# KRLabsOrg/verbatim-rag

Hardware: AMD Instinct MI355X
Metric: query x chunk span-extractions/sec @512tok (ModernBERT-base extractor, chunks/s) (higher is better)
Workload: dtype bf16

## Files before the change

verbatim-rag_amd/csrc/qkv_attn.hip:

```cpp
#include "qkv_attn.h"

#include <cstdlib>
#include <type_traits>

#ifdef VRAG_DEBUG_API
#define VRAG_DBG(bit) ((p.debug_flags & (bit)) != 0)
#else
#define VRAG_DBG(bit) false
#endif

namespace vrag {

constexpr int QA_WB = 192 * 128;
constexpr int QA_XOFF = 2 * QA_WB;
constexpr int QA_TAB = 131072;
constexpr int QA_MU = QA_TAB, QA_RS = QA_TAB + 2048, QA_LS = QA_TAB + 4096;
constexpr int QA_CA = QA_TAB + 5120, QA_SA = QA_CA + 4096, QA_CB = QA_SA + 4096, QA_SB = QA_CB + 2048;
constexpr int QA_SMEM = QA_SB + 2048;
constexpr int QA_V_OFF = 65536;

constexpr float QA_LAZY = 8.0f;
__device__ __forceinline__ float max3f(float a, float b, float c) { return __builtin_fmaxf(__builtin_fmaxf(a, b), c); }

template <int N>
__device__ __forceinline__ void wait_vm() {
  asm volatile("s_waitcnt vmcnt(%0)" ::"n"(N) : "memory");
}

template <bool LOCAL, bool FOLD, typename T>
__global__ __launch_bounds__(512, 2) void qkv_attn_kernel(const QkvAttnParams p) {
  typedef typename Op<T>::v4 V4;
  typedef typename Op<T>::v8 V8;
  extern __shared__ __attribute__((aligned(16))) char smem[];
  const int tid = threadIdx.x;
  const int lane = tid & 63;
  const int wave = uniform(tid >> 6);
  const int g = lane >> 4, l15 = lane & 15;
  const int H = p.H, Tp = p.Tp, nh = p.nh;
  const int xcd = blockIdx.x & 7, slot = blockIdx.x >> 3;
  const int grp = (slot / nh) * 8 + xcd, head = slot % nh;
  if (grp >= p.n_groups) return;
  const int4 wd = p.groups[grp * 8 + wave];
  const int wrow0 = uniform(wd.x), S = uniform(wd.y), kbase = uniform(wd.z);
  const int srow0 = wave * 64;
  const int qrow0 = (wave - kbase) * 64;
  const bool active = qrow0 < S;
  const T* X = reinterpret_cast<const T*>(p.x);
  const T* Wh = reinterpret_cast<const T*>(p.w) + (size_t)head * 192 * H;

  unsigned voffX[2], voffW[3];
#pragma unroll
  for (int par = 0; par < 2; ++par) {
    const int r = par * 8 + (lane >> 3);
    voffX[par] = (unsigned)(r * H + (((lane & 7) ^ ((r >> 1) & 7)) << 3)) * 2u;
  }
#pragma unroll
  for (int i = 0; i < 3; ++i) {
    const int row = wave * 24 + i * 8 + (lane >> 3);
    voffW[i] = (unsigned)(row * H + (((lane & 7) ^ ((row >> 1) & 7)) << 3)) * 2u;
  }
  const char* const Xw = reinterpret_cast<const char*>(X + (size_t)wrow0 * H);
  const char* const Wb = reinterpret_cast<const char*>(Wh);
  char* const xbuf = smem + QA_XOFF + wave * 8192;
  auto dma_w = [&](int kt, int buf, int i) {
    if (VRAG_DBG(4)) return;
    unsigned vo = voffW[i];
    asm volatile("" : "+v"(vo));
    glds16(Wb + kt * 128 + vo, smem + buf * QA_WB + (wave * 24 + i * 8) * 128);
  };
  auto dma_x = [&](int kt, int i) {
    if (!active || VRAG_DBG(4)) return;
    unsigned vo = voffX[i & 1];
    asm volatile("" : "+v"(vo));
    glds16(Xw + ((size_t)(i >> 1) * 16 * H + kt * 64) * 2 + vo, xbuf + i * 1024);
  };

  if (!VRAG_DBG(4)) {
    if (FOLD && lane < 16) {
      glds16(p.ln_mu + min(wrow0 + lane * 4, Tp - 4), smem + QA_MU + srow0 * 4);
      glds16(p.ln_rstd + min(wrow0 + lane * 4, Tp - 4), smem + QA_RS + srow0 * 4);
    }
    if (FOLD && wave == 2) glds16(p.ln_s + head * 192 + lane * 4, smem + QA_LS);
    if (wave == 2 || wave == 3) {
      const float* tab = wave == 2 ? p.rope_cos : p.rope_sin;
#pragma unroll
      for (int i = 0; i < 2; ++i) {
        const int r = i * 8 + (lane >> 3);
        glds16(tab + min(r, p.rope_rows - 1) * 32 + (((lane & 7) ^ ((r >> 1) & 7)) << 2), smem + (wave == 2 ? QA_CB : QA_SB) + i * 1024);
      }
    }
    if (wave == 4 || wave == 5) {
      const float* tab = wave == 4 ? p.rope_cos : p.rope_sin;
#pragma unroll
      for (int i = 0; i < 4; ++i)
        glds16(tab + (size_t)min(16 * (i * 8 + (lane >> 3)), p.rope_rows - 1) * 32 + (lane & 7) * 4, smem + (wave == 4 ? QA_CA : QA_SA) + i * 1024);
    }
  }

  f32x4 acc[12][4];
#pragma unroll
  for (int a = 0; a < 12; ++a)
#pragma unroll
    for (int c = 0; c < 4; ++c) acc[a][c] = f32x4{0.f, 0.f, 0.f, 0.f};

  const int KT = H >> 6;
  int fo[2];
#pragma unroll
  for (int s2 = 0; s2 < 2; ++s2) fo[s2] = l15 * 128 + ((((4 * s2 + g) ^ ((l15 >> 1) & 7))) << 4);
#ifdef VRAG_DEBUG_API
  const int probe = p.debug_flags;
#else
  int probe = 0;
  asm volatile("" : "+s"(probe));
#endif
  const bool mm = active && !(probe & 2);
#pragma unroll
  for (int i = 0; i < 3; ++i) dma_w(0, 0, i);
#pragma unroll
  for (int i = 0; i < 8; ++i) dma_x(0, i);
  for (int kt = 0; kt < KT; ++kt) {
    wait_vm<0>();
    __builtin_amdgcn_s_barrier();
    asm volatile("" ::: "memory");
    const char* sW = smem + (kt & 1) * QA_WB;
    const bool more = kt + 1 < KT;
    V8 xf[2][4], wa;
    if (mm) {
#pragma unroll
      for (int s2 = 0; s2 < 2; ++s2)
#pragma unroll
        for (int rt = 0; rt < 4; ++rt) xf[s2][rt] = *reinterpret_cast<const V8*>(xbuf + rt * 16 * 128 + fo[s2]);
      wa = *reinterpret_cast<const V8*>(sW + fo[0]);
    }
    asm volatile("s_waitcnt lgkmcnt(0)" ::: "memory");
    __builtin_amdgcn_sched_barrier(0);
    if (mm) {
#pragma unroll
      for (int it = 0; it < 24; ++it) {
        const int s2 = it / 12, nj = it % 12;
        V8 na = wa;
        if (it < 23) na = *reinterpret_cast<const V8*>(sW + ((it + 1) % 12) * 16 * 128 + fo[(it + 1) / 12]);
        __builtin_amdgcn_sched_barrier(0);
#pragma unroll
        for (int rt = 0; rt < 4; ++rt) {
          if (nj < 8) acc[nj][rt] = Op<T>::mfma16(wa, xf[s2][rt], acc[nj][rt]);
          else acc[nj][rt] = Op<T>::mfma16(xf[s2][rt], wa, acc[nj][rt]);
        }
        __builtin_amdgcn_sched_barrier(0);
        if (more && it < 11) {
          if (it < 3) dma_w(kt + 1, (kt + 1) & 1, it);
          else dma_x(kt + 1, it - 3);
        }
        __builtin_amdgcn_sched_barrier(0);
        wa = na;
      }
    } else if (more) {
#pragma unroll
      for (int i = 0; i < 3; ++i) dma_w(kt + 1, (kt + 1) & 1, i);
#pragma unroll
      for (int i = 0; i < 8; ++i) dma_x(kt + 1, i);
    }
  }
  __syncthreads();
  if (VRAG_DBG(16)) return;

  const float* l_mu = reinterpret_cast<const float*>(smem + QA_MU) + srow0;
  const float* l_rs = reinterpret_cast<const float*>(smem + QA_RS) + srow0;
  const float* l_ls = reinterpret_cast<const float*>(smem + QA_LS);
#pragma unroll
  for (int db = 0; db < 4; ++db) {
    const int d = db * 16 + l15;
    const float lsv = FOLD ? l_ls[128 + d] : 0.f;
#pragma unroll
    for (int tp = 0; tp < 2; ++tp) {
      V8 vv;
#pragma unroll
      for (int a = 0; a < 2; ++a) {
        const int rt = 2 * tp + a;
        f32x4 m4 = {0.f, 0.f, 0.f, 0.f}, r4 = {1.f, 1.f, 1.f, 1.f};
        if constexpr (FOLD) {
          m4 = *reinterpret_cast<const f32x4*>(l_mu + rt * 16 + 4 * g);
          r4 = *reinterpret_cast<const f32x4*>(l_rs + rt * 16 + 4 * g);
        }
#pragma unroll
        for (int h = 0; h < 2; ++h) {
          const int r0 = 2 * h;
          const f32x2 v = pk_fma(f32x2{-m4[r0], -m4[r0 + 1]}, splat2(lsv), f32x2{acc[8 + db][rt][r0], acc[8 + db][rt][r0 + 1]}) * f32x2{r4[r0], r4[r0 + 1]};
#pragma unroll
          for (int e = 0; e < 2; ++e)
            vv[a * 4 + r0 + e] = qrow0 + rt * 16 + 4 * g + r0 + e < S ? Op<T>::to(v[e]) : (T)0.f;
        }
      }
      const int c = wave * 8 + tp * 4 + g;
      *reinterpret_cast<V8*>(smem + QA_V_OFF + d * 1024 + ((c ^ l15) << 4)) = vv;
    }
  }
  auto rope_rows = [&](int a0, int rt, int ls_off, float scale, V8 (&out)[2]) {
    const bool live = qrow0 + rt * 16 + l15 < S;
    const float mu = FOLD ? l_mu[rt * 16 + l15] : 0.f, rs = FOLD ? l_rs[rt * 16 + l15] : 1.f;
#pragma unroll
    for (int np = 0; np < 2; ++np) {
      const int dd = np * 16 + 4 * g;
      const f32x4 ca = *reinterpret_cast<const f32x4*>(smem + QA_CA + (((qrow0 >> 4) + rt) * 32 + dd) * 4);
      const f32x4 sa = *reinterpret_cast<const f32x4*>(smem + QA_SA + (((qrow0 >> 4) + rt) * 32 + dd) * 4);
      const int bsw = l15 * 128 + ((((dd >> 2) ^ ((l15 >> 1) & 7))) << 4);
      const f32x4 cb = *reinterpret_cast<const f32x4*>(smem + QA_CB + bsw);
      const f32x4 sb = *reinterpret_cast<const f32x4*>(smem + QA_SB + bsw);
      f32x4 l1 = {0.f, 0.f, 0.f, 0.f}, l2 = {0.f, 0.f, 0.f, 0.f};
      if constexpr (FOLD) {
        l1 = *reinterpret_cast<const f32x4*>(l_ls + ls_off + dd);
        l2 = *reinterpret_cast<const f32x4*>(l_ls + ls_off + 32 + dd);
      }
#pragma unroll
      for (int h = 0; h < 2; ++h) {
        const int j0 = 2 * h;
        f32x2 x1 = {acc[a0 + np][rt][j0], acc[a0 + np][rt][j0 + 1]}, x2 = {acc[a0 + 2 + np][rt][j0], acc[a0 + 2 + np][rt][j0 + 1]};
        if constexpr (FOLD) {
          x1 = pk_fma(splat2(-mu), f32x2{l1[j0], l1[j0 + 1]}, x1) * rs;
          x2 = pk_fma(splat2(-mu), f32x2{l2[j0], l2[j0 + 1]}, x2) * rs;
        }
        const f32x2 ca2 = {ca[j0], ca[j0 + 1]}, sa2 = {sa[j0], sa[j0 + 1]}, cb2 = {cb[j0], cb[j0 + 1]}, sb2 = {sb[j0], sb[j0 + 1]};
        const f32x2 c = pk_fma(-sa2, sb2, ca2 * cb2), sn = pk_fma(ca2, sb2, sa2 * cb2);
        const f32x2 o1 = pk_fma(-x2, sn, x1 * c) * scale, o2 = pk_fma(x1, sn, x2 * c) * scale;
#pragma unroll
        for (int e = 0; e < 2; ++e) {
          if constexpr (!std::is_same<T, bf16_t>::value) {
            out[0][np * 4 + j0 + e] = live ? Op<T>::to(o1[e]) : (T)0.f;
            out[1][np * 4 + j0 + e] = live ? Op<T>::to(o2[e]) : (T)0.f;
          } else {
            out[0][np * 4 + j0 + e] = Op<T>::to(o1[e]);
            out[1][np * 4 + j0 + e] = Op<T>::to(o2[e]);
          }
        }
      }
    }
  };
#pragma unroll
  for (int rt = 0; rt < 4; ++rt) {
    V8 kf[2];
    rope_rows(4, rt, 64, 1.0f, kf);
    const int row = srow0 + rt * 16 + l15;
#pragma unroll
    for (int s = 0; s < 2; ++s) *reinterpret_cast<V8*>(smem + row * 128 + (((4 * s + g) ^ ((row >> 1) & 7)) << 4)) = kf[s];
  }
  V8 qf[4][2];
#pragma unroll
  for (int rt = 0; rt < 4; ++rt) rope_rows(0, rt, 0, p.q_scale, qf[rt]);
  __syncthreads();

  f32x4 ot[4][4];
  f32x4 lo[4];
#pragma unroll
  for (int c = 0; c < 4; ++c) {
    lo[c] = f32x4{0.f, 0.f, 0.f, 0.f};
#pragma unroll
    for (int dt = 0; dt < 4; ++dt) ot[c][dt] = f32x4{0.f, 0.f, 0.f, 0.f};
  }
  float m_run[4] = {0.f, 0.f, 0.f, 0.f};
  bool seen[4] = {false, false, false, false};
  V8 ones;
#pragma unroll
  for (int j = 0; j < 8; ++j) ones[j] = (T)1.0f;
  const int W = p.window;
  int kt_lo = 0, kt_hi = (S - 1) >> 6;
  if constexpr (LOCAL) {
    kt_lo = max(0, qrow0 - W) >> 6;
    kt_hi = min(S - 1, qrow0 + 63 + W) >> 6;
  }
  const int ksw = (l15 >> 1) & 7;
  if (active && !VRAG_DBG(1)) {
    for (int kt = kt_lo; kt <= kt_hi; ++kt) {
      bool cut[2][2];
#pragma unroll
      for (int u = 0; u < 2; ++u) {
        const int q_lo = qrow0 + 32 * u;
#pragma unroll
        for (int t2 = 0; t2 < 2; ++t2) {
          const int kh = kt * 64 + t2 * 32;
          bool outside = kh >= S || q_lo >= S;
          cut[u][t2] = kh + 31 >= S;
          if constexpr (LOCAL) {
            outside = outside || (kh + 31 < q_lo - W) || (kh > q_lo + 31 + W);
            cut[u][t2] = cut[u][t2] || (kh < q_lo + 31 - W) || (kh + 31 > q_lo + W);
          }
          cut[u][t2] = cut[u][t2] || outside;
        }
      }
      V8 pf[4][2];
      {
        f32x4 st[4][4];
#pragma unroll
        for (int c = 0; c < 4; ++c) {
          const float seed = -m_run[c];
#pragma unroll
          for (int kb = 0; kb < 4; ++kb) st[c][kb] = f32x4{seed, seed, seed, seed};
        }
#pragma unroll
        for (int kb = 0; kb < 4; ++kb) {
          const char* krow = smem + ((kbase + kt) * 64 + kb * 16 + l15) * 128;
          const V8 k0 = *reinterpret_cast<const V8*>(krow + ((g ^ ksw) << 4));
          const V8 k1 = *reinterpret_cast<const V8*>(krow + (((4 + g) ^ ksw) << 4));
#pragma unroll
          for (int c = 0; c < 4; ++c) {
            st[c][kb] = Op<T>::mfma16(k0, qf[c][0], st[c][kb]);
            st[c][kb] = Op<T>::mfma16(k1, qf[c][1], st[c][kb]);
          }
        }
        float mx[4];
#pragma unroll
        for (int c = 0; c < 4; ++c) {
          const int u = c >> 1;
          mx[c] = -INFINITY;
#pragma unroll
          for (int t2 = 0; t2 < 2; ++t2) {
            if (cut[u][t2]) {
              const int qi = qrow0 + 16 * c + l15;
              int lo_k = 0, hi_k = S - 1;
              if constexpr (LOCAL) {
                lo_k = max(0, qi - W);
                hi_k = min(S - 1, qi + W);
              }
              const unsigned span = hi_k >= lo_k ? (unsigned)(hi_k - lo_k) : 0u;
              int d0 = hi_k >= lo_k ? kt * 64 + t2 * 32 + 4 * g - lo_k : -100000;
              asm volatile("" : "+v"(d0));
#pragma unroll
              for (int h2 = 0; h2 < 2; ++h2)
#pragma unroll
                for (int r = 0; r < 4; ++r) {
                  const bool ok = (unsigned)(d0 + 16 * h2 + r) <= span;
                  st[c][2 * t2 + h2][r] = ok ? st[c][2 * t2 + h2][r] : -INFINITY;
                }
            }
            const f32x4& a = st[c][2 * t2];
            const f32x4& b2 = st[c][2 * t2 + 1];
            mx[c] = max3f(mx[c], max3f(a[0], a[1], a[2]), max3f(a[3], b2[0], b2[1]));
            mx[c] = max3f(mx[c], b2[2], b2[3]);
          }
        }
        bool move = false;
#pragma unroll
        for (int c = 0; c < 4; ++c) move = move || mx[c] > QA_LAZY || (!seen[c] && mx[c] > -INFINITY);
        if (__any(move)) {
#pragma unroll
          for (int c = 0; c < 4; ++c) {
            float m_all = fmaxf(mx[c], __shfl_xor(mx[c], 16, 64));
            m_all = fmaxf(m_all, __shfl_xor(m_all, 32, 64));
            const bool has = m_all > -INFINITY;
            const float delta = seen[c] ? fmaxf(m_all, 0.f) : (has ? m_all : 0.f);
            const float alpha = seen[c] ? __builtin_amdgcn_exp2f(-delta) : 1.0f;
            seen[c] = seen[c] || has;
            m_run[c] += delta;
#pragma unroll
            for (int kb = 0; kb < 4; ++kb)
#pragma unroll
              for (int r = 0; r < 4; ++r) st[c][kb][r] -= delta;
#pragma unroll
            for (int dt = 0; dt < 4; ++dt)
#pragma unroll
              for (int r = 0; r < 4; ++r) ot[c][dt][r] *= alpha;
#pragma unroll
            for (int r = 0; r < 4; ++r) lo[c][r] *= alpha;
          }
        }
#pragma unroll
        for (int c = 0; c < 4; ++c)
#pragma unroll
          for (int t2 = 0; t2 < 2; ++t2)
#pragma unroll
            for (int j = 0; j < 8; ++j) pf[c][t2][j] = (T)__builtin_amdgcn_exp2f(st[c][2 * t2 + (j >> 2)][j & 3]);
      }
#pragma unroll
      for (int t2 = 0; t2 < 2; ++t2) {
#pragma unroll
        for (int c = 0; c < 4; ++c) lo[c] = Op<T>::mfma16(ones, pf[c][t2], lo[c]);
#pragma unroll
        for (int dt = 0; dt < 4; ++dt) {
          const V8 vf = *reinterpret_cast<const V8*>(smem + QA_V_OFF + (dt * 16 + l15) * 1024 + ((((kbase + kt) * 8 + t2 * 4 + g) ^ l15) << 4));
#pragma unroll
          for (int c = 0; c < 4; ++c) ot[c][dt] = Op<T>::mfma16(vf, pf[c][t2], ot[c][dt]);
        }
      }
    }
  }
  __syncthreads();

  if (active) {
    char* stg = smem + wave * 8192;
#pragma unroll
    for (int rt = 0; rt < 4; ++rt) {
      const int row = rt * 16 + l15;
      const bool live = qrow0 + row < S;
      const float inv = live ? 1.0f / lo[rt][0] : 0.f;
#pragma unroll
      for (int db = 0; db < 4; ++db) {
        V4 o;
#pragma unroll
        for (int j = 0; j < 4; ++j) o[j] = live ? Op<T>::to(ot[rt][db][j] * inv) : (T)0.f;
        const int c16 = db * 2 + (g >> 1);
        *reinterpret_cast<V4*>(stg + row * 128 + ((c16 ^ (row & 7)) << 4) + ((g & 1) << 3)) = o;
      }
    }
#pragma unroll
    for (int it = 0; it < 8; ++it) {
      const int row = it * 8 + (lane >> 3), c16 = lane & 7;
      const f32x4 v = *reinterpret_cast<const f32x4*>(stg + row * 128 + ((c16 ^ (row & 7)) << 4));
      if (qrow0 + row < S && !VRAG_DBG(8)) store16_nt(reinterpret_cast<T*>(p.o) + (size_t)(wrow0 + row) * H + head * 64 + c16 * 8, v);
    }
  }
}

template <bool LOCAL, bool FOLD, typename T>
static hipError_t launch_t(const QkvAttnParams& p, hipStream_t stream) {
  static bool attr = false;
  if (!attr) {
    hipError_t e = hipFuncSetAttribute(reinterpret_cast<const void*>(&qkv_attn_kernel<LOCAL, FOLD, T>),
                                       hipFuncAttributeMaxDynamicSharedMemorySize, QA_SMEM);
    if (e != hipSuccess) return e;
    attr = true;
  }
  const int grid = ((p.n_groups + 7) / 8) * 8 * p.nh;
  hipLaunchKernelGGL((qkv_attn_kernel<LOCAL, FOLD, T>), dim3(grid), dim3(512), QA_SMEM, stream, p);
  return hipGetLastError();
}

hipError_t launch_qkv_attention(const QkvAttnParams& p, bool local, hipStream_t stream) {
  if (p.n_groups <= 0) return hipSuccess;
  if (p.H % 64 != 0 || p.H != p.nh * 64 || (size_t)p.Tp * p.H >= (size_t)1 << 31) return hipErrorInvalidValue;
  const bool fold = p.ln_mu != nullptr;
  if (p.op_dtype == kOpF16) {
    if (fold) return local ? launch_t<true, true, f16_t>(p, stream) : launch_t<false, true, f16_t>(p, stream);
    return local ? launch_t<true, false, f16_t>(p, stream) : launch_t<false, false, f16_t>(p, stream);
  }
  if (fold) return local ? launch_t<true, true, bf16_t>(p, stream) : launch_t<false, true, bf16_t>(p, stream);
  return local ? launch_t<true, false, bf16_t>(p, stream) : launch_t<false, false, bf16_t>(p, stream);
}

__global__ void permute_qkv_heads_kernel(const bf16_t* __restrict__ w, const float* __restrict__ s, int H, int nh,
                                         bf16_t* __restrict__ w_out, float* __restrict__ s_out) {
  const int orow = blockIdx.x;
  const int head = orow / 192, part = (orow % 192) / 64, d = orow % 64;
  const int src = part * H + head * 64 + d;
  for (int i = threadIdx.x; i < H; i += blockDim.x) w_out[(size_t)orow * H + i] = w[(size_t)src * H + i];
  if (threadIdx.x == 0 && s && s_out) s_out[orow] = s[src];
}

hipError_t permute_qkv_heads(const bf16_t* w, const float* s, int H, int nh, bf16_t* w_out, float* s_out, hipStream_t stream) {
  hipLaunchKernelGGL(permute_qkv_heads_kernel, dim3(3 * H), dim3(256), 0, stream, w, s, H, nh, w_out, s_out);
  return hipGetLastError();
}

int fused_pack_groups(const int* seq_row, const int* seq_len, int seq0, int seq1, int4* out) {
  int n = 0, used = 8;
  for (int s = seq0; s < seq1; ++s) {
    const int need = (seq_len[s] + 63) / 64;
    if (used + need > 8) {
      for (int w = 0; w < 8; ++w) out[n * 8 + w] = int4{0, 0, 0, 0};
      ++n;
      used = 0;
    }
    for (int j = 0; j < need; ++j) out[(n - 1) * 8 + used + j] = int4{seq_row[s] + 64 * j, seq_len[s], used, 0};
    used += need;
  }
  return n;
}

unsigned qkv_attn_f16_saturated(bool reset) { return f16_sat_take(reset); }
unsigned* qkv_attn_f16_flag_address() { return f16_sat_flag_address(); }

}
```

Before: 7633.

## Skip dead attention sub-blocks at local-window edges and specialize full-tile epilogue

Splits the key-tile loop in local (sliding-window) attention so the first and last tiles use compile-time specializations that skip MFMA, masking, exp and PV work for 32x32 sub-blocks entirely outside the window. The V/K/Q rope epilogue is also templated on whether the query tile is fully in-bounds, removing per-element bounds selects for full bf16 folded tiles, and the q scale is folded into the row scale multiply. This adds code size and register pressure from multiple instantiations.

```diff
diff --git a/verbatim-rag_amd/csrc/qkv_attn.hip b/verbatim-rag_amd/csrc/qkv_attn.hip
--- a/verbatim-rag_amd/csrc/qkv_attn.hip
+++ b/verbatim-rag_amd/csrc/qkv_attn.hip
@@ -167,85 +167,93 @@
   const float* l_mu = reinterpret_cast<const float*>(smem + QA_MU) + srow0;
   const float* l_rs = reinterpret_cast<const float*>(smem + QA_RS) + srow0;
   const float* l_ls = reinterpret_cast<const float*>(smem + QA_LS);
-#pragma unroll
-  for (int db = 0; db < 4; ++db) {
-    const int d = db * 16 + l15;
-    const float lsv = FOLD ? l_ls[128 + d] : 0.f;
-#pragma unroll
-    for (int tp = 0; tp < 2; ++tp) {
-      V8 vv;
-#pragma unroll
-      for (int a = 0; a < 2; ++a) {
-        const int rt = 2 * tp + a;
-        f32x4 m4 = {0.f, 0.f, 0.f, 0.f}, r4 = {1.f, 1.f, 1.f, 1.f};
+  V8 qf[4][2];
+  auto epilogue = [&](auto all_c) __attribute__((always_inline)) {
+    constexpr bool ALL = decltype(all_c)::value;
+#pragma unroll
+    for (int db = 0; db < 4; ++db) {
+      const int d = db * 16 + l15;
+      const float lsv = FOLD ? l_ls[128 + d] : 0.f;
+#pragma unroll
+      for (int tp = 0; tp < 2; ++tp) {
+        V8 vv;
+#pragma unroll
+        for (int a = 0; a < 2; ++a) {
+          const int rt = 2 * tp + a;
+          f32x4 m4 = {0.f, 0.f, 0.f, 0.f}, r4 = {1.f, 1.f, 1.f, 1.f};
+          if constexpr (FOLD) {
+            m4 = *reinterpret_cast<const f32x4*>(l_mu + rt * 16 + 4 * g);
+            r4 = *reinterpret_cast<const f32x4*>(l_rs + rt * 16 + 4 * g);
+          }
+#pragma unroll
+          for (int h = 0; h < 2; ++h) {
+            const int r0 = 2 * h;
+            const f32x2 v = pk_fma(f32x2{-m4[r0], -m4[r0 + 1]}, splat2(lsv), f32x2{acc[8 + db][rt][r0], acc[8 + db][rt][r0 + 1]}) * f32x2{r4[r0], r4[r0 + 1]};
+#pragma unroll
+            for (int e = 0; e < 2; ++e)
+              vv[a * 4 + r0 + e] = ALL || qrow0 + rt * 16 + 4 * g + r0 + e < S ? Op<T>::to(v[e]) : (T)0.f;
+          }
+        }
+        const int c = wave * 8 + tp * 4 + g;
+        *reinterpret_cast<V8*>(smem + QA_V_OFF + d * 1024 + ((c ^ l15) << 4)) = vv;
+      }
+    }
+    auto rope_rows = [&](int a0, int rt, int ls_off, float scale, V8 (&out)[2]) {
+      const bool live = ALL || qrow0 + rt * 16 + l15 < S;
+      const float mu = FOLD ? l_mu[rt * 16 + l15] : 0.f, rs = FOLD ? l_rs[rt * 16 + l15] * scale : scale;
+#pragma unroll
+      for (int np = 0; np < 2; ++np) {
+        const int dd = np * 16 + 4 * g;
+        const f32x4 ca = *reinterpret_cast<const f32x4*>(smem + QA_CA + (((qrow0 >> 4) + rt) * 32 + dd) * 4);
+        const f32x4 sa = *reinterpret_cast<const f32x4*>(smem + QA_SA + (((qrow0 >> 4) + rt) * 32 + dd) * 4);
+        const int bsw = l15 * 128 + ((((dd >> 2) ^ ((l15 >> 1) & 7))) << 4);
+        const f32x4 cb = *reinterpret_cast<const f32x4*>(smem + QA_CB + bsw);
+        const f32x4 sb = *reinterpret_cast<const f32x4*>(smem + QA_SB + bsw);
+        f32x4 l1 = {0.f, 0.f, 0.f, 0.f}, l2 = {0.f, 0.f, 0.f, 0.f};
         if constexpr (FOLD) {
-          m4 = *reinterpret_cast<const f32x4*>(l_mu + rt * 16 + 4 * g);
-          r4 = *reinterpret_cast<const f32x4*>(l_rs + rt * 16 + 4 * g);
+          l1 = *reinterpret_cast<const f32x4*>(l_ls + ls_off + dd);
+          l2 = *reinterpret_cast<const f32x4*>(l_ls + ls_off + 32 + dd);
         }
 #pragma unroll
         for (int h = 0; h < 2; ++h) {
-          const int r0 = 2 * h;
-          const f32x2 v = pk_fma(f32x2{-m4[r0], -m4[r0 + 1]}, splat2(lsv), f32x2{acc[8 + db][rt][r0], acc[8 + db][rt][r0 + 1]}) * f32x2{r4[r0], r4[r0 + 1]};
-#pragma unroll
-          for (int e = 0; e < 2; ++e)
-            vv[a * 4 + r0 + e] = qrow0 + rt * 16 + 4 * g + r0 + e < S ? Op<T>::to(v[e]) : (T)0.f;
-        }
-      }
-      const int c = wave * 8 + tp * 4 + g;
-      *reinterpret_cast<V8*>(smem + QA_V_OFF + d * 1024 + ((c ^ l15) << 4)) = vv;
-    }
-  }
-  auto rope_rows = [&](int a0, int rt, int ls_off, float scale, V8 (&out)[2]) {
-    const bool live = qrow0 + rt * 16 + l15 < S;
-    const float mu = FOLD ? l_mu[rt * 16 + l15] : 0.f, rs = FOLD ? l_rs[rt * 16 + l15] : 1.f;
-#pragma unroll
-    for (int np = 0; np < 2; ++np) {
-      const int dd = np * 16 + 4 * g;
-      const f32x4 ca = *reinterpret_cast<const f32x4*>(smem + QA_CA + (((qrow0 >> 4) + rt) * 32 + dd) * 4);
-      const f32x4 sa = *reinterpret_cast<const f32x4*>(smem + QA_SA + (((qrow0 >> 4) + rt) * 32 + dd) * 4);
-      const int bsw = l15 * 128 + ((((dd >> 2) ^ ((l15 >> 1) & 7))) << 4);
-      const f32x4 cb = *reinterpret_cast<const f32x4*>(smem + QA_CB + bsw);
-      const f32x4 sb = *reinterpret_cast<const f32x4*>(smem + QA_SB + bsw);
-      f32x4 l1 = {0.f, 0.f, 0.f, 0.f}, l2 = {0.f, 0.f, 0.f, 0.f};
-      if constexpr (FOLD) {
-        l1 = *reinterpret_cast<const f32x4*>(l_ls + ls_off + dd);
-        l2 = *reinterpret_cast<const f32x4*>(l_ls + ls_off + 32 + dd);
-      }
-#pragma unroll
-      for (int h = 0; h < 2; ++h) {
-        const int j0 = 2 * h;
-        f32x2 x1 = {acc[a0 + np][rt][j0], acc[a0 + np][rt][j0 + 1]}, x2 = {acc[a0 + 2 + np][rt][j0], acc[a0 + 2 + np][rt][j0 + 1]};
-        if constexpr (FOLD) {
-          x1 = pk_fma(splat2(-mu), f32x2{l1[j0], l1[j0 + 1]}, x1) * rs;
-          x2 = pk_fma(splat2(-mu), f32x2{l2[j0], l2[j0 + 1]}, x2) * rs;
-        }
-        const f32x2 ca2 = {ca[j0], ca[j0 + 1]}, sa2 = {sa[j0], sa[j0 + 1]}, cb2 = {cb[j0], cb[j0 + 1]}, sb2 = {sb[j0], sb[j0 + 1]};
-        const f32x2 c = pk_fma(-sa2, sb2, ca2 * cb2), sn = pk_fma(ca2, sb2, sa2 * cb2);
-        const f32x2 o1 = pk_fma(-x2, sn, x1 * c) * scale, o2 = pk_fma(x1, sn, x2 * c) * scale;
-#pragma unroll
-        for (int e = 0; e < 2; ++e) {
-          if constexpr (!std::is_same<T, bf16_t>::value) {
-            out[0][np * 4 + j0 + e] = live ? Op<T>::to(o1[e]) : (T)0.f;
-            out[1][np * 4 + j0 + e] = live ? Op<T>::to(o2[e]) : (T)0.f;
-          } else {
-            out[0][np * 4 + j0 + e] = Op<T>::to(o1[e]);
-            out[1][np * 4 + j0 + e] = Op<T>::to(o2[e]);
+          const int j0 = 2 * h;
+          f32x2 x1 = {acc[a0 + np][rt][j0], acc[a0 + np][rt][j0 + 1]}, x2 = {acc[a0 + 2 + np][rt][j0], acc[a0 + 2 + np][rt][j0 + 1]};
+          if constexpr (FOLD) {
+            x1 = pk_fma(splat2(-mu), f32x2{l1[j0], l1[j0 + 1]}, x1) * rs;
+            x2 = pk_fma(splat2(-mu), f32x2{l2[j0], l2[j0 + 1]}, x2) * rs;
+          } else if (scale != 1.0f) {
+            x1 = x1 * rs;
+            x2 = x2 * rs;
           }
-        }
-      }
-    }
+          const f32x2 ca2 = {ca[j0], ca[j0 + 1]}, sa2 = {sa[j0], sa[j0 + 1]}, cb2 = {cb[j0], cb[j0 + 1]}, sb2 = {sb[j0], sb[j0 + 1]};
+          const f32x2 c = pk_fma(-sa2, sb2, ca2 * cb2), sn = pk_fma(ca2, sb2, sa2 * cb2);
+          const f32x2 o1 = pk_fma(-x2, sn, x1 * c), o2 = pk_fma(x1, sn, x2 * c);
+#pragma unroll
+          for (int e = 0; e < 2; ++e) {
+            if constexpr (!std::is_same<T, bf16_t>::value) {
+              out[0][np * 4 + j0 + e] = live ? Op<T>::to(o1[e]) : (T)0.f;
+              out[1][np * 4 + j0 + e] = live ? Op<T>::to(o2[e]) : (T)0.f;
+            } else {
+              out[0][np * 4 + j0 + e] = Op<T>::to(o1[e]);
+              out[1][np * 4 + j0 + e] = Op<T>::to(o2[e]);
+            }
+          }
+        }
+      }
+    };
+#pragma unroll
+    for (int rt = 0; rt < 4; ++rt) {
+      V8 kf[2];
+      rope_rows(4, rt, 64, 1.0f, kf);
+      const int row = srow0 + rt * 16 + l15;
+#pragma unroll
+      for (int s = 0; s < 2; ++s) *reinterpret_cast<V8*>(smem + row * 128 + (((4 * s + g) ^ ((row >> 1) & 7)) << 4)) = kf[s];
+    }
+#pragma unroll
+    for (int rt = 0; rt < 4; ++rt) rope_rows(0, rt, 0, p.q_scale, qf[rt]);
   };
-#pragma unroll
-  for (int rt = 0; rt < 4; ++rt) {
-    V8 kf[2];
-    rope_rows(4, rt, 64, 1.0f, kf);
-    const int row = srow0 + rt * 16 + l15;
-#pragma unroll
-    for (int s = 0; s < 2; ++s) *reinterpret_cast<V8*>(smem + row * 128 + (((4 * s + g) ^ ((row >> 1) & 7)) << 4)) = kf[s];
-  }
-  V8 qf[4][2];
-#pragma unroll
-  for (int rt = 0; rt < 4; ++rt) rope_rows(0, rt, 0, p.q_scale, qf[rt]);
+  if (FOLD && std::is_same<T, bf16_t>::value && qrow0 + 64 <= S) epilogue(std::true_type{});
+  else epilogue(std::false_type{});
   __syncthreads();
 
   f32x4 ot[4][4];
@@ -268,117 +276,154 @@
     kt_hi = min(S - 1, qrow0 + 63 + W) >> 6;
   }
   const int ksw = (l15 >> 1) & 7;
+  auto tile = [&](int kt, const bool (&cut)[2][2], auto dead_c) __attribute__((always_inline)) {
+    constexpr int DEAD = decltype(dead_c)::value;
+    auto live_blk = [](int u, int t2) constexpr { return !(DEAD == 1 && u == 1 && t2 == 0) && !(DEAD == 2 && u == 0 && t2 == 1); };
+    V8 pf[4][2];
+    {
+      f32x4 st[4][4];
+#pragma unroll
+      for (int c = 0; c < 4; ++c) {
+        const float seed = -m_run[c];
+#pragma unroll
+        for (int kb = 0; kb < 4; ++kb) st[c][kb] = f32x4{seed, seed, seed, seed};
+      }
+#pragma unroll
+      for (int kb = 0; kb < 4; ++kb) {
+        const char* krow = smem + ((kbase + kt) * 64 + kb * 16 + l15) * 128;
+        const V8 k0 = *reinterpret_cast<const V8*>(krow + ((g ^ ksw) << 4));
+        const V8 k1 = *reinterpret_cast<const V8*>(krow + (((4 + g) ^ ksw) << 4));
+#pragma unroll
+        for (int c = 0; c < 4; ++c) {
+          if (!live_blk(c >> 1, kb >> 1)) continue;
+          st[c][kb] = Op<T>::mfma16(k0, qf[c][0], st[c][kb]);
+          st[c][kb] = Op<T>::mfma16(k1, qf[c][1], st[c][kb]);
+        }
+      }
+      float mx[4];
+#pragma unroll
+      for (int c = 0; c < 4; ++c) {
+        const int u = c >> 1;
+        mx[c] = -INFINITY;
+#pragma unroll
+        for (int t2 = 0; t2 < 2; ++t2) {
+          if (!live_blk(u, t2)) continue;
+          if (cut[u][t2]) {
+            const int qi = qrow0 + 16 * c + l15;
+            int lo_k = 0, hi_k = S - 1;
+            if constexpr (LOCAL) {
+              lo_k = max(0, qi - W);
+              hi_k = min(S - 1, qi + W);
+            }
+            const unsigned span = hi_k >= lo_k ? (unsigned)(hi_k - lo_k) : 0u;
+            int d0 = hi_k >= lo_k ? kt * 64 + t2 * 32 + 4 * g - lo_k : -100000;
+            asm volatile("" : "+v"(d0));
+#pragma unroll
+            for (int h2 = 0; h2 < 2; ++h2)
+#pragma unroll
+              for (int r = 0; r < 4; ++r) {
+                const bool ok = (unsigned)(d0 + 16 * h2 + r) <= span;
+                st[c][2 * t2 + h2][r] = ok ? st[c][2 * t2 + h2][r] : -INFINITY;
+              }
+          }
+          const f32x4& a = st[c][2 * t2];
+          const f32x4& b2 = st[c][2 * t2 + 1];
+          mx[c] = max3f(mx[c], max3f(a[0], a[1], a[2]), max3f(a[3], b2[0], b2[1]));
+          mx[c] = max3f(mx[c], b2[2], b2[3]);
+        }
+      }
+      bool move = false;
+#pragma unroll
+      for (int c = 0; c < 4; ++c) move = move || mx[c] > QA_LAZY || (!seen[c] && mx[c] > -INFINITY);
+      if (__any(move)) {
+#pragma unroll
+        for (int c = 0; c < 4; ++c) {
+          float m_all = fmaxf(mx[c], __shfl_xor(mx[c], 16, 64));
+          m_all = fmaxf(m_all, __shfl_xor(m_all, 32, 64));
+          const bool has = m_all > -INFINITY;
+          const float delta = seen[c] ? fmaxf(m_all, 0.f) : (has ? m_all : 0.f);
+          const float alpha = seen[c] ? __builtin_amdgcn_exp2f(-delta) : 1.0f;
+          seen[c] = seen[c] || has;
+          m_run[c] += delta;
+#pragma unroll
+          for (int kb = 0; kb < 4; ++kb)
+#pragma unroll
+            for (int r = 0; r < 4; ++r)
+              if (live_blk(c >> 1, kb >> 1)) st[c][kb][r] -= delta;
+#pragma unroll
+          for (int dt = 0; dt < 4; ++dt)
+#pragma unroll
+            for (int r = 0; r < 4; ++r) ot[c][dt][r] *= alpha;
+#pragma unroll
+          for (int r = 0; r < 4; ++r) lo[c][r] *= alpha;
+        }
+      }
+#pragma unroll
+      for (int c = 0; c < 4; ++c)
+#pragma unroll
+        for (int t2 = 0; t2 < 2; ++t2)
+#pragma unroll
+          for (int j = 0; j < 8; ++j)
+            if (live_blk(c >> 1, t2)) pf[c][t2][j] = (T)__builtin_amdgcn_exp2f(st[c][2 * t2 + (j >> 2)][j & 3]);
+    }
+#pragma unroll
+    for (int t2 = 0; t2 < 2; ++t2) {
+#pragma unroll
+      for (int c = 0; c < 4; ++c)
+        if (live_blk(c >> 1, t2)) lo[c] = Op<T>::mfma16(ones, pf[c][t2], lo[c]);
+#pragma unroll
+      for (int dt = 0; dt < 4; ++dt) {
+        const V8 vf = *reinterpret_cast<const V8*>(smem + QA_V_OFF + (dt * 16 + l15) * 1024 + ((((kbase + kt) * 8 + t2 * 4 + g) ^ l15) << 4));
+#pragma unroll
+        for (int c = 0; c < 4; ++c)
+          if (live_blk(c >> 1, t2)) ot[c][dt] = Op<T>::mfma16(vf, pf[c][t2], ot[c][dt]);
+      }
+    }
+  };
+  auto blocks = [&](int kt, bool (&cut)[2][2], bool (&outside_blk)[2][2]) __attribute__((always_inline)) {
+#pragma unroll
+    for (int u = 0; u < 2; ++u) {
+      const int q_lo = qrow0 + 32 * u;
+#pragma unroll
+      for (int t2 = 0; t2 < 2; ++t2) {
+        const int kh = kt * 64 + t2 * 32;
+        bool outside = kh >= S || q_lo >= S;
+        cut[u][t2] = kh + 31 >= S;
+        if constexpr (LOCAL) {
+          outside = outside || (kh + 31 < q_lo - W) || (kh > q_lo + 31 + W);
+          cut[u][t2] = cut[u][t2] || (kh < q_lo + 31 - W) || (kh + 31 > q_lo + W);
+        }
+        cut[u][t2] = cut[u][t2] || outside;
+        outside_blk[u][t2] = outside;
+      }
+    }
+  };
   if (active && !VRAG_DBG(1)) {
-    for (int kt = kt_lo; kt <= kt_hi; ++kt) {
-      bool cut[2][2];
-#pragma unroll
-      for (int u = 0; u < 2; ++u) {
-        const int q_lo = qrow0 + 32 * u;
-#pragma unroll
-        for (int t2 = 0; t2 < 2; ++t2) {
-          const int kh = kt * 64 + t2 * 32;
-          bool outside = kh >= S || q_lo >= S;
-          cut[u][t2] = kh + 31 >= S;
-          if constexpr (LOCAL) {
-            outside = outside || (kh + 31 < q_lo - W) || (kh > q_lo + 31 + W);
-            cut[u][t2] = cut[u][t2] || (kh < q_lo + 31 - W) || (kh + 31 > q_lo + W);
-          }
-          cut[u][t2] = cut[u][t2] || outside;
-        }
-      }
-      V8 pf[4][2];
-      {
-        f32x4 st[4][4];
-#pragma unroll
-        for (int c = 0; c < 4; ++c) {
-          const float seed = -m_run[c];
-#pragma unroll
-          for (int kb = 0; kb < 4; ++kb) st[c][kb] = f32x4{seed, seed, seed, seed};
-        }
-#pragma unroll
-        for (int kb = 0; kb < 4; ++kb) {
-          const char* krow = smem + ((kbase + kt) * 64 + kb * 16 + l15) * 128;
-          const V8 k0 = *reinterpret_cast<const V8*>(krow + ((g ^ ksw) << 4));
-          const V8 k1 = *reinterpret_cast<const V8*>(krow + (((4 + g) ^ ksw) << 4));
-#pragma unroll
-          for (int c = 0; c < 4; ++c) {
-            st[c][kb] = Op<T>::mfma16(k0, qf[c][0], st[c][kb]);
-            st[c][kb] = Op<T>::mfma16(k1, qf[c][1], st[c][kb]);
-          }
-        }
-        float mx[4];
-#pragma unroll
-        for (int c = 0; c < 4; ++c) {
-          const int u = c >> 1;
-          mx[c] = -INFINITY;
-#pragma unroll
-          for (int t2 = 0; t2 < 2; ++t2) {
-            if (cut[u][t2]) {
-              const int qi = qrow0 + 16 * c + l15;
-              int lo_k = 0, hi_k = S - 1;
-              if constexpr (LOCAL) {
-                lo_k = max(0, qi - W);
-                hi_k = min(S - 1, qi + W);
-              }
-              const unsigned span = hi_k >= lo_k ? (unsigned)(hi_k - lo_k) : 0u;
-              int d0 = hi_k >= lo_k ? kt * 64 + t2 * 32 + 4 * g - lo_k : -100000;
-              asm volatile("" : "+v"(d0));
-#pragma unroll
-              for (int h2 = 0; h2 < 2; ++h2)
-#pragma unroll
-                for (int r = 0; r < 4; ++r) {
-                  const bool ok = (unsigned)(d0 + 16 * h2 + r) <= span;
-                  st[c][2 * t2 + h2][r] = ok ? st[c][2 * t2 + h2][r] : -INFINITY;
-                }
-            }
-            const f32x4& a = st[c][2 * t2];
-            const f32x4& b2 = st[c][2 * t2 + 1];
-            mx[c] = max3f(mx[c], max3f(a[0], a[1], a[2]), max3f(a[3], b2[0], b2[1]));
-            mx[c] = max3f(mx[c], b2[2], b2[3]);
-          }
-        }
-        bool move = false;
-#pragma unroll
-        for (int c = 0; c < 4; ++c) move = move || mx[c] > QA_LAZY || (!seen[c] && mx[c] > -INFINITY);
-        if (__any(move)) {
-#pragma unroll
-          for (int c = 0; c < 4; ++c) {
-            float m_all = fmaxf(mx[c], __shfl_xor(mx[c], 16, 64));
-            m_all = fmaxf(m_all, __shfl_xor(m_all, 32, 64));
-            const bool has = m_all > -INFINITY;
-            const float delta = seen[c] ? fmaxf(m_all, 0.f) : (has ? m_all : 0.f);
-            const float alpha = seen[c] ? __builtin_amdgcn_exp2f(-delta) : 1.0f;
-            seen[c] = seen[c] || has;
-            m_run[c] += delta;
-#pragma unroll
-            for (int kb = 0; kb < 4; ++kb)
-#pragma unroll
-              for (int r = 0; r < 4; ++r) st[c][kb][r] -= delta;
-#pragma unroll
-            for (int dt = 0; dt < 4; ++dt)
-#pragma unroll
-              for (int r = 0; r < 4; ++r) ot[c][dt][r] *= alpha;
-#pragma unroll
-            for (int r = 0; r < 4; ++r) lo[c][r] *= alpha;
-          }
-        }
-#pragma unroll
-        for (int c = 0; c < 4; ++c)
-#pragma unroll
-          for (int t2 = 0; t2 < 2; ++t2)
-#pragma unroll
-            for (int j = 0; j < 8; ++j) pf[c][t2][j] = (T)__builtin_amdgcn_exp2f(st[c][2 * t2 + (j >> 2)][j & 3]);
-      }
-#pragma unroll
-      for (int t2 = 0; t2 < 2; ++t2) {
-#pragma unroll
-        for (int c = 0; c < 4; ++c) lo[c] = Op<T>::mfma16(ones, pf[c][t2], lo[c]);
-#pragma unroll
-        for (int dt = 0; dt < 4; ++dt) {
-          const V8 vf = *reinterpret_cast<const V8*>(smem + QA_V_OFF + (dt * 16 + l15) * 1024 + ((((kbase + kt) * 8 + t2 * 4 + g) ^ l15) << 4));
-#pragma unroll
-          for (int c = 0; c < 4; ++c) ot[c][dt] = Op<T>::mfma16(vf, pf[c][t2], ot[c][dt]);
-        }
+    bool cut[2][2], outside_blk[2][2];
+    int kt = kt_lo;
+    if constexpr (LOCAL) {
+      blocks(kt, cut, outside_blk);
+      if (outside_blk[1][0]) {
+        tile(kt, cut, std::integral_constant<int, 1>{});
+        ++kt;
+      }
+    }
+    int kt_end = kt_hi;
+    if constexpr (LOCAL) {
+      if (kt <= kt_hi) {
+        blocks(kt_hi, cut, outside_blk);
+        if (outside_blk[0][1]) --kt_end;
+      }
+    }
+    for (int k2 = kt; k2 <= kt_end; ++k2) {
+      bool c2[2][2], o2[2][2];
+      blocks(k2, c2, o2);
+      tile(k2, c2, std::integral_constant<int, 0>{});
+    }
+    if constexpr (LOCAL) {
+      if (kt_end < kt_hi) {
+        blocks(kt_hi, cut, outside_blk);
+        tile(kt_hi, cut, std::integral_constant<int, 2>{});
       }
     }
   }
```

New measurement: 7692, median of 6. Within noise of the previous version (+0.8%).
